# MadNLP/MadQP.jl

Measured on AMD Instinct MI355X. Metric: IPM iterations/sec (Mehrotra predictor-corrector, condensed KKT + Cholesky), dense QP fp64; value = steps / time of the timed iterations, initialize! excluded (value_reference_definition: iter / total_time), higher is better.
Workload: dtype f64

## Files before the change

__graft_entry__.py:

```python
import os
import subprocess
import sys

ROOT = os.path.dirname(os.path.abspath(__file__))
if ROOT not in sys.path:
    sys.path.insert(0, ROOT)


def build() -> None:
    subprocess.check_call(["make", "-C", os.path.join(ROOT, "madqp_jl_amd", "csrc"), "-j8"])
    subprocess.check_call(["make", "-C", os.path.join(ROOT, "tests", "csrc")])
    subprocess.check_call(["make", "-C", os.path.join(ROOT, "tests", "csrc_band")])
    subprocess.check_call(["make", "-C", os.path.join(ROOT, "tests", "csrc_solve")])
    import madqp_jl_amd as M

    lib = M.load_cdll()
    assert lib.madqp_version() == 100
    for name in M.EXPORTED_SYMBOLS:
        getattr(lib, name)


def smoke() -> None:
    import numpy as np

    import madqp_jl_amd as M
    from oracle import mpc
    from oracle import qp as Q

    be = M.HipBackend(0)
    qp = Q.synthetic_qp(20250614, 300, 120)
    dq = M.DeviceQP.from_numpy(be.device, qp.H, qp.q, qp.A, qp.lvar, qp.uvar, qp.lcon, qp.ucon, qp.x0)
    s = M.MPCSolver(dq, be, regularization=M.FixedRegularization(1e-8, -1e-8))
    r = s.solve()
    ref = mpc.solve(qp, kkt_system="condensed", regularization=mpc.FixedRegularization(1e-8, -1e-8))
    assert r["status"] == ref["status"] == M.SOLVE_SUCCEEDED, (r["status"], ref["status"])
    assert r["iter"] == ref["iter"], (r["iter"], ref["iter"])
    assert abs(r["objective"] - ref["objective"]) <= 1e-9 * max(1.0, abs(ref["objective"]))
    assert np.max(np.abs(r["solution"] - ref["solution"])) <= 1e-7
    for a, b in zip(r["trace"], ref["trace"]):
        tol = 1e-9 if min(a["mu"], b["mu"]) >= 1e-4 else 1e-6
        for k in ("alpha_p", "alpha_d", "inf_pr", "inf_du"):
            assert abs(a[k] - b[k]) <= tol * max(1.0, abs(b[k])), (a["k"], k, a[k], b[k])
    print(f"smoke ok: {r['iter']} iterations, objective {r['objective']:.12e}, "
          f"fp64 MFMA probe {be.probe_mfma_f64(100000):.1f} TFLOP/s")
    s.kkt.close()
    be.close()


if __name__ == "__main__":
    build()
    if len(sys.argv) > 1 and sys.argv[1] == "smoke":
        smoke()
```

madqp_jl_amd/csrc/chol.hip:

```cpp
#include <algorithm>
#include <cstdlib>

#include <vector>

#include "common.h"
#include "band_plan.inc"
#include "mid_plan.inc"
#include "solve_plan.inc"

typedef double double2_t __attribute__((ext_vector_type(2)));

namespace {
constexpr int NB = 128;
constexpr int NBO = 1024;
static_assert(SOLVE_NB == NB, "solve_plan.inc plans in this file's blocks");
constexpr int64_t SOLVE_MANY_MIN_DEFAULT = 32;
#ifndef P2_LDS_LD
#define P2_LDS_LD (NB + 1)
#endif
constexpr int LDS_LD = P2_LDS_LD;
constexpr int64_t WBLK = 2 * NB * NB;

typedef double double4_t __attribute__((ext_vector_type(4)));
#include "gemm_core.inc"
// ... 823 lines not shown
        }
}
template <int J>
__device__ __forceinline__ void ps16_step(double4_t (&z)[8], const double (&aw)[4], const double (&al)[7][4]) {
    double4_t t = {0.0, 0.0, 0.0, 0.0};
#pragma unroll
    for (int s = 0; s < 4; ++s) t = __builtin_amdgcn_mfma_f64_16x16x4f64(aw[s], z[J][s], t, 0, 0, 0);
    z[J] = t;
#pragma unroll
    for (int d = 0; d < 7; ++d)
        if (J + 1 + d < 8) {
#pragma unroll
            for (int s = 0; s < 4; ++s)
                z[J + 1 + d] = __builtin_amdgcn_mfma_f64_16x16x4f64(al[d][s], t[s], z[J + 1 + d], 0, 0, 0);
        }
}
__device__ __forceinline__ void panel_sub16_body(double* __restrict__ C, int64_t ld, const double* __restrict__ Lkk,
                                                 int64_t ldl, const double* __restrict__ Wcm, int64_t rows, int64_t rows_read) {
    const int lane = threadIdx.x & 63, wave = __builtin_amdgcn_readfirstlane(threadIdx.x >> 6);
    const int lo = lane & 15, hi = lane >> 4;
    const int64_t i0 = (int64_t)blockIdx.x * 64 + wave * 16;
    if (i0 >= rows) return;
    const int64_t gi = i0 + lo;
    const int64_t gir = gi < rows_read ? gi : rows_read - 1;
    double* Cp = C + gir + (int64_t)hi * ld;
    const double* Lq = Lkk + lo + (int64_t)hi * ldl;
    const double* Wq = Wcm + lo + hi * NB;
    double aw[3][4], al[3][7][4];
    ps16_load<0>(Lq, ldl, Wq, aw[0], al[0]);
    ps16_load<1>(Lq, ldl, Wq, aw[1], al[1]);
    double4_t z[8];
#pragma unroll
    for (int J = 0; J < 8; ++J)
#pragma unroll
        for (int v = 0; v < 4; ++v) z[J][v] = -Cp[(int64_t)(16 * J + 4 * v) * ld];
    ps16_load<2>(Lq, ldl, Wq, aw[2], al[2]);
    ps16_step<0>(z, aw[0], al[0]);
    ps16_load<3>(Lq, ldl, Wq, aw[0], al[0]);
    ps16_step<1>(z, aw[1], al[1]);
    ps16_load<4>(Lq, ldl, Wq, aw[1], al[1]);
    ps16_step<2>(z, aw[2], al[2]);
    ps16_load<5>(Lq, ldl, Wq, aw[2], al[2]);
    ps16_step<3>(z, aw[0], al[0]);
    ps16_load<6>(Lq, ldl, Wq, aw[0], al[0]);
    ps16_step<4>(z, aw[1], al[1]);
    ps16_load<7>(Lq, ldl, Wq, aw[1], al[1]);
    ps16_step<5>(z, aw[2], al[2]);
    ps16_step<6>(z, aw[0], al[0]);
    ps16_step<7>(z, aw[1], al[1]);
    if (gi < rows) {
        double* Co = C + gi + (int64_t)hi * ld;
#pragma unroll
        for (int J = 0; J < 8; ++J)
#pragma unroll
            for (int v = 0; v < 4; ++v) Co[(int64_t)(16 * J + 4 * v) * ld] = z[J][v];
    }
}

__global__ __launch_bounds__(256) void panel_sub16_kernel(double* __restrict__ C, int64_t ld, const double* __restrict__ Lkk,
                                                          int64_t ldl, const double* __restrict__ Wcm, int64_t rows,
                                                          int64_t rows_read, PanelBatch bt) {
    if (bt.list) {
        const int cnt = *bt.count;
        for (int pb = blockIdx.y; pb < cnt; pb += gridDim.y) {
            const int64_t b = bt.list[pb];
            panel_sub16_body(C + b * bt.sC, ld, Lkk + b * bt.sL, ldl, Wcm + b * bt.sW, rows, rows_read);
        }
        return;
    }
    if (gridDim.y > 1 || bt.skip) {
        const int64_t b = blockIdx.y;
        if (bt.skip && bt.skip[b] != 0) return;
        C += b * bt.sC;
        Lkk += b * bt.sL;
        Wcm += b * bt.sW;
    }
    panel_sub16_body(C, ld, Lkk, ldl, Wcm, rows, rows_read);
}

struct MidArgs {
    double* A;
    int64_t lda, n;
    int32_t nblk, k;
    const uint32_t* plan;
    double* winv;
    int32_t* info;
};
#ifdef MADQP_MID_STAMPS
__device__ unsigned long long madqp_mid_stamps[64][24];
#define MID_STAMP(slot)                                                                                              \
    do {                                                                                                             \
        if (threadIdx.x == 0 && blockIdx.x <= 2)                                                                     \
            madqp_mid_stamps[a.k & 63][8 * blockIdx.x + (slot)] = __builtin_amdgcn_s_memrealtime();                  \
    } while (0)
#else
#define MID_STAMP(slot)
#endif
constexpr int MID_THREADS = 512;

constexpr int XS_LD = 144;
static_assert(NB * XS_LD <= P2_S_DOUBLES + P2_WD_DOUBLES, "the operand image fits the diagonal kernel's LDS");
#ifdef MADQP_MID_STAMPS
#define DS_STAMP(slot)                                                                                   \
    do {                                                                                                 \
        if (threadIdx.x == 0) madqp_mid_stamps[kstep & 63][(slot)] = __builtin_amdgcn_s_memrealtime();   \
    } while (0)
#else
#define DS_STAMP(slot)
#endif
__device__ __forceinline__ void mid_diag_syrk(const double* __restrict__ Ckk, const double* __restrict__ R, int64_t lda, int nb,
                                              double* __restrict__ smem, int kstep) {
    const int tid = threadIdx.x, lane = tid & 63, wave = __builtin_amdgcn_readfirstlane(tid >> 6);
    const int lo = lane & 15, hi = lane >> 4;
    const int p = wave >> 1, first = (wave & 1) ? 5 : 0, cnt = (wave & 1) ? 4 : 5;
    int tI[5], tJ[5];
#pragma unroll
    for (int u = 0; u < 5; ++u) {
        int q = first + (u < cnt ? u : cnt - 1);
        tI[u] = (q <= p) ? p : 7 - p;
        tJ[u] = (q <= p) ? q : q - (p + 1);
    }
    double2_t rv[16];
#pragma unroll
    for (int q = 0; q < 16; ++q) {
        const int e = tid + MID_THREADS * q, c = e >> 6, i = 2 * (e & 63);
        rv[q] = *reinterpret_cast<const double2_t*>(R + i + (int64_t)c * lda);
    }
    double4_t acc[5];
#pragma unroll
    for (int u = 0; u < 5; ++u)
#pragma unroll
        for (int v = 0; v < 4; ++v) {
            int c = 16 * tJ[u] + hi + 4 * v;
            c = c < nb ? c : nb - 1;
            acc[u][v] = -Ckk[(16 * tI[u] + lo) + (int64_t)c * lda];
        }
#pragma unroll
    for (int q = 0; q < 16; ++q) {
        const int e = tid + MID_THREADS * q, c = e >> 6, i = 2 * (e & 63);
        *reinterpret_cast<double2_t*>(smem + c * XS_LD + i) = rv[q];
    }
    __syncthreads();
    DS_STAMP(4);
    const double* xa[5];
    const double* xb[5];
#pragma unroll
    for (int u = 0; u < 5; ++u) {
        xa[u] = smem + hi * XS_LD + 16 * tJ[u] + lo;
        xb[u] = smem + hi * XS_LD + 16 * tI[u] + lo;
    }
#pragma unroll 2
    for (int s4 = 0; s4 < 32; ++s4) {
#pragma unroll
        for (int u = 0; u < 5; ++u)
            acc[u] = __builtin_amdgcn_mfma_f64_16x16x4f64(xa[u][4 * s4 * XS_LD], xb[u][4 * s4 * XS_LD], acc[u], 0, 0, 0);
    }
    DS_STAMP(5);
    __syncthreads();
    DS_STAMP(6);
#pragma unroll
    for (int u = 0; u < 5; ++u) {
        if (u >= cnt) continue;
#pragma unroll
        for (int v = 0; v < 4; ++v) {
            const int r = 16 * tI[u] + lo, c = 16 * tJ[u] + hi + 4 * v;
            double x = -acc[u][v];
            if (r >= nb || c >= nb) x = (r == c) ? 1.0 : 0.0;
            smem[c * LDS_LD + r] = (r >= c) ? x : 0.0;
        }
    }
    __syncthreads();
}

__global__ __launch_bounds__(MID_THREADS) void chol_mid_step_kernel(MidArgs a) {
    __shared__ __attribute__((aligned(16))) double smem[P2_S_DOUBLES + P2_WD_DOUBLES];
    static_assert(P2_S_DOUBLES + P2_WD_DOUBLES >= 4 * TILE_DOUBLES, "the GEMM stages fit the diagonal kernel's LDS");
    const int tid = threadIdx.x, lane = tid & 63;
    const int wave = __builtin_amdgcn_readfirstlane(tid >> 6);
    const int k = a.k;
    MID_STAMP(0);
    if (blockIdx.x == 0) {
        const int64_t i0 = (int64_t)k * NB;
        const int nb = (int)((a.n - i0 < NB) ? (a.n - i0) : NB);
        double* Akk = a.A + i0 + i0 * a.lda;
        if (k > 0) mid_diag_syrk(Akk, a.A + i0 + (int64_t)(k - 1) * NB * a.lda, a.lda, nb, smem, k);
        MID_STAMP(1);
        MID_STAMP(2);
        double* Wcm = a.winv + (int64_t)k * WBLK;
        potf2_inv_body<MID_THREADS, 1>(Akk, a.lda, nb, Wcm, Wcm + NB * NB, a.info, (int32_t)i0, smem, smem + P2_S_DOUBLES,
                                       k > 0);
        MID_STAMP(3);
        return;
    }
    const uint32_t e = a.plan[(int)blockIdx.x - 1];
    const int bi = __builtin_amdgcn_readfirstlane((int)(e & 255u));
    const int bj = __builtin_amdgcn_readfirstlane((int)((e >> 8) & 255u));
    const int pan0 = __builtin_amdgcn_readfirstlane((int)((e >> 16) & 255u));
    const int kpan = __builtin_amdgcn_readfirstlane((int)(e >> 24));
    const int64_t i0 = (int64_t)bi * NB, j0 = (int64_t)bj * NB;
    if (wave >= 4) {
        const int nbar = kpan * (NB / BK) + 1;
        for (int b = 0; b < nbar; ++b) __builtin_amdgcn_s_barrier();
        return;
    }
    const int wi = wave & 1, wj = wave >> 1;
    const int lo = lane & 15, hi = lane >> 4;
    GemmArgs g{};
    g.X = a.A + (int64_t)pan0 * NB * a.lda;
    g.Y = g.X;
    g.ldx = g.ldy = a.lda;
    g.M = g.N = a.n;
    g.Mread = g.Nread = (int64_t)a.nblk * NB;
    g.K = kpan * NB;
    double4_t acc[4][4];
#pragma unroll
    for (int ti = 0; ti < 4; ++ti)
#pragma unroll
        for (int tj = 0; tj < 4; ++tj)
#pragma unroll
            for (int v = 0; v < 4; ++v) {
                int64_t gj = j0 + wj * 64 + tj * 16 + hi + 4 * v;
                gj = (gj < a.n) ? gj : a.n - 1;
                acc[ti][tj][v] = -a.A[i0 + wi * 64 + ti * 16 + lo + gj * a.lda];
            }
    mainloop_dma(g, i0, j0, smem, wi, wj, lane, wave, acc);
    MID_STAMP(1);
#pragma unroll
    for (int ti = 0; ti < 4; ++ti) {
        const int64_t gi = i0 + wi * 64 + ti * 16 + lo;
#pragma unroll
        for (int tj = 0; tj < 4; ++tj) {
#pragma unroll
            for (int v = 0; v < 4; ++v) {
                const int64_t gj = j0 + wj * 64 + tj * 16 + hi + 4 * v;
                if (gi < a.n && gj < a.n && gi >= gj) a.A[gi + gj * a.lda] = -acc[ti][tj][v];
            }
        }
    }
    MID_STAMP(7);
}

}

struct CholModes {
    bool sweep_upper;
    int32_t sweep_chunk;
    bool sweep_band;
    int64_t mid_max;
    int mid_cap;
    int64_t wt_min, wt_max;
    int64_t band_w;
};
static CholModes chol_modes_from_env() {
    auto num = [](const char* name, int64_t dflt) { return getenv(name) ? atoll(getenv(name)) : dflt; };
    auto on = [&](const char* name) { return num(name, 1) != 0; };
    CholModes m{};
    m.sweep_upper = on("MADQP_SWEEP_UPPER");
    m.sweep_chunk = (int32_t)std::max<int64_t>(1, num("MADQP_SWEEP_CHUNK", 64));
    m.sweep_band = on("MADQP_SWEEP_BAND");
    m.mid_max = num("MADQP_CHOL_MID_MAX", 13312);
    m.mid_cap = (int)num("MADQP_CHOL_MID_CAP", 0);
    m.wt_min = num("MADQP_CHOL_WMIN", 6);
    m.wt_max = num("MADQP_CHOL_WMAX", 20);
    m.band_w = std::max<int64_t>(0, num("MADQP_CHOL_BAND_W", 0));
    return m;
}
static const CholModes& chol_modes() {
    static const CholModes m = chol_modes_from_env();
    return m;
}

static hipError_t band_clear(madqp_chol* s) {
    const hipError_t e = s->mem.free_one(&s->band.d_jobs);
    s->band = madqp_chol_band{};
    s->band.extent = s->n - 1;
    return e;
}
static int32_t adopt_matrix(madqp_chol* s, double* A, int64_t lda) {
    ARG_TRY(s->ctx, A && lda >= (s->band.packed ? std::max<int64_t>(s->band.extent, 1) : s->n));
    s->A = A;
    s->lda = lda;
    s->upper_ok = false;
    return MADQP_OK;
}
static void forget_factor(madqp_chol* s) {
    s->A = nullptr;
    s->upper_ok = false;
}

extern "C" int32_t madqp_chol_create(madqp_ctx* ctx, int64_t n, madqp_chol** out) {
    ARG_TRY(ctx, ctx && out && n >= 0);
    *out = nullptr;
    madqp_chol* s = new (std::nothrow) madqp_chol();
    if (!s) return madqp_fail(ctx, MADQP_ERR_ALLOC, "host allocation failed");
    s->ctx = s->mem.ctx = ctx;
    s->n = s->npos = n;
    s->band.extent = n - 1;
    s->many_min = SOLVE_MANY_MIN_DEFAULT;
    const int64_t nblk = std::max<int64_t>(1, (n + NB - 1) / NB);
    const CholModes md = chol_modes_from_env();
    s->sweep_chunk = md.sweep_chunk;
    s->sweep_band = md.sweep_band;
    std::vector<int32_t> jobs;
    if (nblk - 1 > s->sweep_chunk && nblk < (1 << 20)) {
        s->sweep_maxc = (int32_t)band_sweep_jobs(nblk, -1, s->sweep_chunk, jobs);
        s->sweep_njobs = (int32_t)jobs.size();
    }
    s->tmp_len = nblk * NB + 2 * nblk * (int64_t)s->sweep_maxc * NB;
    s->utmp_len = nblk * NB + s->tmp_len;
    const bool with_x = nblk > 1 && nblk <= 160;
    const char* who = "madqp_chol_create";
    auto hip_ok = [&](hipError_t e) {
        return e == hipSuccess ? MADQP_OK : madqp_fail(ctx, MADQP_ERR_ALLOC, "madqp_chol_create(%lld): %s", (long long)n, hipGetErrorString(e));
    };
    int32_t r = s->mem.alloc(&s->winv, nblk * WBLK, who);
    if (!r) r = hip_ok(hipMemset(s->winv, 0, nblk * WBLK * sizeof(double)));
    double* scratch = nullptr;
    if (!r) r = s->mem.alloc(&scratch, with_x ? s->utmp_len : s->tmp_len, who);
    s->sweep_x = with_x ? scratch : nullptr;
    s->sweep_y = with_x && scratch ? scratch + nblk * NB : scratch;
    if (!r && !jobs.empty()) {
        r = s->mem.alloc(&s->d_jobs, (int64_t)jobs.size(), who);
        if (!r) r = hip_ok(hipMemcpy(s->d_jobs, jobs.data(), jobs.size() * sizeof(int32_t), hipMemcpyHostToDevice));
    }
    if (!r) r = s->mem.alloc(&s->d_info, 8, who);
    if (r) {
        madqp_chol_destroy(s);
        return r;
    }
    *out = s;
    return MADQP_OK;
}

static int64_t handle_plan(const madqp_chol* s, int64_t bw, std::vector<CholOp>& ops) {
    return chol_plan(s->n, bw < 0 ? s->n - 1 : bw, s->npos, s->ctx->gemm_slots, ops, chol_modes().wt_min, chol_modes().wt_max, chol_modes().band_w);
}

extern "C" int32_t madqp_chol_set_signature(madqp_chol* s, int64_t npos) {
    if (!s) return MADQP_ERR_ARG;
    ARG_TRY(s->ctx, npos >= 0 && npos <= s->n && (npos % NB == 0 || npos == s->n));
    ARG_TRY(s->ctx, s->band.bw < 0 || npos == s->n);
    s->npos = npos;
    s->plan.clear();
    return MADQP_OK;
}

extern "C" int32_t madqp_chol_destroy(madqp_chol* s) {
    if (!s) return MADQP_OK;
    (void)hipStreamSynchronize(s->ctx->stream);
    delete s;
    return MADQP_OK;
}

extern "C" int32_t madqp_chol_set_bandwidth(madqp_chol* s, int64_t bw) {
    if (!s) return MADQP_ERR_ARG;
    madqp_ctx* ctx = s->ctx;
    ARG_TRY(ctx, bw == -1 || (bw >= 0 && bw < s->n && s->npos == s->n));
    forget_factor(s);
    if (s->band.d_jobs) HIP_TRY(ctx, hipStreamSynchronize(ctx->stream));
    HIP_TRY(ctx, band_clear(s));
    s->plan.clear();
    if (bw < 0) return MADQP_OK;
    madqp_chol_band b;
    b.bw = bw;
    b.extent = handle_plan(s, bw, s->plan);
    if (s->sweep_band) {
        b.sweep_kb = band_sweep_blocks(bw);
        if (s->d_jobs) {
            std::vector<int32_t> jobs;
            band_sweep_jobs((s->n + NB - 1) / NB, b.sweep_kb, s->sweep_chunk, jobs);
            const size_t before = s->mem.owned.size();
            int32_t r = s->mem.alloc(&b.d_jobs, (int64_t)jobs.size(), "madqp_chol_set_bandwidth");
            const hipError_t e = r ? hipSuccess : hipMemcpy(b.d_jobs, jobs.data(), jobs.size() * sizeof(int32_t), hipMemcpyHostToDevice);
            if (e != hipSuccess) r = madqp_fail(ctx, MADQP_ERR_ALLOC, "madqp_chol_set_bandwidth: %s", hipGetErrorString(e));
            if (r) {
                s->mem.release(before);
                s->plan.clear();
                return r;
            }
            b.njobs = (int32_t)jobs.size();
        }
    }
    s->band = b;
    return MADQP_OK;
}

extern "C" int32_t madqp_chol_sweep_info(madqp_chol* s, int64_t* out_host) {
    if (!s || !out_host) return MADQP_ERR_ARG;
    const bool band = s->band.sweep_kb >= 0;
    const int64_t nblk = std::max<int64_t>(1, (s->n + NB - 1) / NB);
    out_host[0] = band ? s->band.sweep_kb : -1;
    out_host[1] = !s->d_jobs ? nblk : band ? s->band.njobs : s->sweep_njobs;
    out_host[2] = s->sweep_chunk;
    return MADQP_OK;
}

extern "C" int32_t madqp_chol_band_extent(madqp_chol* s, int64_t* extent_host) {
    if (!s) return MADQP_ERR_ARG;
    ARG_TRY(s->ctx, extent_host != nullptr);
    *extent_host = s->band.extent;
    return MADQP_OK;
}

static int64_t packed_ld_pad() {
    const char* e = getenv("MADQP_BAND_LD_PAD");
    return e ? std::max<int64_t>(0, atoll(e)) / 2 * 2 : BAND_PACKED_PAD;
}
extern "C" int32_t madqp_chol_packed_layout(madqp_chol* s, int64_t ld_in, int64_t* out_host) {
    if (!s) return MADQP_ERR_ARG;
    ARG_TRY(s->ctx, out_host != nullptr && s->band.bw >= 0);
    if (!band_packed_layout(s->n, s->band.extent, ld_in, out_host, packed_ld_pad()))
        return madqp_fail(s->ctx, MADQP_ERR_ARG, "madqp_chol_packed_layout: ld = %lld is below the extent %lld", (long long)ld_in,
                          (long long)s->band.extent);
    return MADQP_OK;
}
extern "C" int32_t madqp_chol_set_packed(madqp_chol* s, int32_t on) {
    if (!s) return MADQP_ERR_ARG;
    ARG_TRY(s->ctx, !on || (s->band.bw >= 0 && s->band.sweep_kb >= 0 && s->npos == s->n));
    if (s->band.packed != (on != 0)) forget_factor(s);
    s->band.packed = on != 0;
    return MADQP_OK;
}

static_assert(BAND_NB == NB && BAND_NBO == NBO, "chol_plan.inc plans in this file's blocks");

struct CholTarget {
    madqp_ctx* ctx;
    double* A;
    int64_t lda, n;
    double* winv;
    int32_t* info;
    bool batched = false;
    int64_t B = 1, sA = 0, sW = 0;
    const int32_t* skip = nullptr;
    const int32_t* list = nullptr;
    const int32_t* count = nullptr;
    bool packed = false;
    int64_t npad() const { return (n + NB - 1) / NB * NB; }
    bool padded() const { return packed || lda >= npad(); }
};
static int32_t target_gemm(const CholTarget& t, const GemmArgs& g, int cls, int64_t sY, int64_t sCin) {
    if (!t.batched) return madqp_gemm_tn(t.ctx, g, cls);
    const GemmBatch bt{t.B, t.sA, sY, t.sA, sCin, 0, t.skip, t.list, t.count};
    return madqp_gemm_tn(t.ctx, g, cls, nullptr, 0, &bt);
}

static int32_t panel_update(const CholTarget& t, const CholOp& o) {
    GemmArgs g{};
    g.X = t.A + o.row0 + o.k0 * t.lda;
    g.ldx = t.lda;
    g.Y = g.X;
    g.ldy = t.lda;
    g.C = t.A + o.row0 + o.row0 * t.lda;
    g.ldc = t.lda;
    g.Cin = g.C;
    g.ldcin = t.lda;
    g.alpha = (double)o.sign;
    g.beta = 1.0;
    g.M = o.rows;
    g.N = o.width;
    g.K = o.kend - o.k0;
    if (t.padded()) {
        g.Mread = (o.rows + NB - 1) / NB * NB;
        g.Nread = std::min<int64_t>(t.npad() - o.row0, (o.width + NB - 1) / NB * NB);
    }
    g.diag_off = 0;
    g.lower_only = 1;
    return target_gemm(t, g, MADQP_PROF_POTRF_GEMM, t.sA, t.sA);
}

static int32_t sweep_images(madqp_chol* s, double* A, int64_t lda, int64_t j0, int64_t w) {
    if (w <= 0) return MADQP_OK;
    madqp_ctx* ctx = s->ctx;
    ProfScope ps(ctx, MADQP_PROF_POTRF_DIAG);
    hipLaunchKernelGGL(sweep_image_kernel, dim3((unsigned)((w + NB - 1) / NB)), dim3(256), 0, ctx->stream, A, lda, s->n, j0, s->winv);
    LAUNCH_CHECK(ctx);
    return MADQP_OK;
}

static const auto sweep_fwd_kernel = trsv_fwd_sweep_kernel<false>;

int32_t madqp_chol_panel_solve(madqp_ctx* ctx, double* X, int64_t ldx, int64_t rows, int64_t rows_read, const double* L,
                               int64_t ldl, const double* Wcm, int64_t w, const CholTarget* batch) {
    if (rows <= 0) return MADQP_OK;
    ARG_TRY(ctx, w == NB);
    ARG_TRY(ctx, rows_read >= rows && (!batch || (batch->B >= 1 && batch->B <= 65535)));
    ProfScope ps(ctx, MADQP_PROF_POTRF_TRSM);
    const PanelBatch bt = batch ? PanelBatch{batch->sA, batch->sA, batch->sW, batch->skip, batch->list, batch->count}
                                : PanelBatch{0, 0, 0, nullptr};
    hipLaunchKernelGGL(panel_sub16_kernel, dim3((unsigned)((rows + 63) / 64), (unsigned)(batch ? batch->B : 1)), dim3(256), 0,
                       ctx->stream, X, ldx, L, ldl, Wcm, rows, rows_read, bt);
    LAUNCH_CHECK(ctx);
    return MADQP_OK;
}

static int32_t factor_block(const CholTarget& t, const CholOp& o) {
    madqp_ctx* ctx = t.ctx;
    const int64_t jb = o.row0, w = o.width, rows = o.rows;
    double* Ajj = t.A + jb + jb * t.lda;
    double* Wcm = t.winv + (jb / NB) * WBLK;
    {
        ProfScope ps(ctx, MADQP_PROF_POTRF_DIAG);
        const Potf2Batch bt = t.batched ? Potf2Batch{t.sA, t.sW, 1, t.skip, t.list, t.count} : Potf2Batch{0, 0, 0, nullptr};
        const auto diag_kernel = t.batched ? potf2_inv_kernel<0> : potf2_inv_kernel<1>;
        hipLaunchKernelGGL(diag_kernel, dim3((unsigned)t.B), dim3(P2_KTHREADS), 0, ctx->stream, Ajj, t.lda, (int)w, Wcm,
                           Wcm + NB * NB, t.info, (int32_t)jb, bt);
        LAUNCH_CHECK(ctx);
    }
    return madqp_chol_panel_solve(ctx, Ajj + w, t.lda, rows, t.padded() ? (rows + NB - 1) / NB * NB : rows, Ajj, t.lda, Wcm, w,
                                  t.batched ? &t : nullptr);
}

static int32_t run_ops(const CholTarget& t, const std::vector<CholOp>& ops) {
    for (const CholOp& o : ops) {
        const int32_t r = o.kind == CHOL_UPDATE ? panel_update(t, o) : factor_block(t, o);
        if (r) return r;
    }
    return MADQP_OK;
}
static CholTarget chol_target(madqp_chol* s, double* A, int64_t lda) {
    CholTarget t{s->ctx, A, lda, s->n, s->winv, s->d_info};
    t.packed = s->band.packed;
    return t;
}

static bool mid_plan_build(madqp_chol* s, int nblk, int cap) {
    MidPlan& mp = s->mid;
    if (mp.state) return mp.state > 0;
    mp.state = -1;
    if (nblk > 255 || cap < 1) return false;
    std::vector<std::vector<MidVisit>> steps;
    std::vector<int32_t> units;
    bool ok = false;
    for (int rounds = 1; rounds <= 64 && !ok; ++rounds) ok = mid_plan_steps(nblk, rounds * cap, steps, units, cap);
    if (!ok) return false;
    std::vector<uint32_t> w;
    std::vector<int32_t> count((size_t)nblk), first((size_t)nblk);
    for (int k = 0; k < nblk; ++k) {
        first[k] = (int32_t)w.size();
        mid_plan_units(nblk, k, steps[k], w);
        count[k] = (int32_t)w.size() - first[k];
        if (count[k] != units[k]) return false;
    }
    if (w.empty()) w.push_back(0);
    const size_t before = s->mem.owned.size();
    uint32_t* d_units = nullptr;
    if (s->mem.alloc(&d_units, (int64_t)w.size(), "madqp_chol_factor: mid-size plan") ||
        hipMemcpy(d_units, w.data(), w.size() * sizeof(uint32_t), hipMemcpyHostToDevice) != hipSuccess) {
        (void)hipGetLastError();
        s->mem.release(before);
        return false;
    }
    mp.count.swap(count);
    mp.first.swap(first);
    mp.d_units = d_units;
    mp.state = 1;
    return true;
}

static int32_t factor_mid(madqp_chol* s, double* A, int64_t lda) {
    madqp_ctx* ctx = s->ctx;
    const int64_t n = s->n;
    const int64_t npad_m = (n + NB - 1) / NB * NB;
    const int32_t nblk = (int32_t)(npad_m / NB);
    ProfScope ps_all(ctx, MADQP_PROF_POTRF_GEMM);
    ProfMute mute(ctx);
    for (int32_t k = 0; k < nblk; ++k) {
        hipLaunchKernelGGL(chol_mid_step_kernel, dim3((unsigned)(1 + s->mid.count[k])), dim3(MID_THREADS), 0, ctx->stream,
                           MidArgs{A, lda, n, nblk, k, s->mid.d_units + s->mid.first[k], s->winv, s->d_info});
        LAUNCH_CHECK(ctx);
        const int64_t jb = (int64_t)k * NB;
        const int32_t r = madqp_chol_panel_solve(ctx, A + (jb + NB) + jb * lda, lda, n - jb - NB, npad_m - jb - NB,
                                                 A + jb + jb * lda, lda, s->winv + (int64_t)k * WBLK, NB);
        if (r) return r;
    }
    const int32_t ri = sweep_images(s, A, lda, 0, n);
    if (ri) return ri;
    if (chol_modes().sweep_upper && s->sweep_x) {
        if (!s->upper) {
            const size_t before = s->mem.owned.size();
            if (s->mem.alloc(&s->upper, npad_m * npad_m, "madqp_chol_factor: U = L'")) {
                s->mem.release(before);
                return MADQP_OK;
            }
            s->upper_ld = npad_m;
        }
        hipLaunchKernelGGL(lower_to_upper_kernel, dim3(2 * nblk, 2 * nblk), dim3(256), 0, ctx->stream, A, lda, n, s->upper,
                           s->upper_ld);
        LAUNCH_CHECK(ctx);
        s->upper_ok = true;
    }
    return MADQP_OK;
}

static int32_t chol_factor_enqueue(madqp_chol* s, double* A, int64_t lda) {
    madqp_ctx* ctx = s->ctx;
    const int64_t n = s->n;
    HIP_TRY(ctx, hipMemsetAsync(s->d_info, 0, sizeof(int32_t), ctx->stream));
    const CholModes& md = chol_modes();
    if (s->band.bw < 0 && n <= md.mid_max && n > NB && s->npos == n && lda >= (n + NB - 1) / NB * NB && lda % 2 == 0 && (((uintptr_t)A) & 15) == 0 &&
        mid_plan_build(s, (int)((n + NB - 1) / NB), md.mid_cap > 0 ? md.mid_cap : ctx->gemm_slots / 2 - 1))
        return factor_mid(s, A, lda);
    if (s->plan.empty()) handle_plan(s, s->band.bw, s->plan);
    const int32_t r = run_ops(chol_target(s, A, lda), s->plan);
    if (r) return r;
    return sweep_images(s, A, lda, 0, n);
}

extern "C" int32_t madqp_chol_factor(madqp_chol* s, double* A, int64_t lda, int32_t* info_host) {
    if (!s) return MADQP_ERR_ARG;
    madqp_ctx* ctx = s->ctx;
    ARG_TRY(ctx, info_host != nullptr);
    int32_t r = adopt_matrix(s, A, lda);
    if (r) return r;
    *info_host = 0;
    if (s->n == 0) return MADQP_OK;
    if ((r = chol_factor_enqueue(s, A, lda))) return r;
    int32_t info = 0;
    HIP_TRY(ctx, hipMemcpyAsync(&info, s->d_info, sizeof(int32_t), hipMemcpyDeviceToHost, ctx->stream));
    HIP_TRY(ctx, hipStreamSynchronize(ctx->stream));
    *info_host = info;
    return MADQP_OK;
}

namespace {
__global__ void info_to_slot_kernel(const int32_t* __restrict__ info, double* __restrict__ slot) {
    *slot = (double)*info;
}
}
int32_t madqp_chol_factor_q(madqp_chol* s, double* A, int64_t lda, double* d_slot) {
    if (!s) return MADQP_ERR_ARG;
    madqp_ctx* ctx = s->ctx;
    ARG_TRY(ctx, d_slot != nullptr);
    int32_t r = adopt_matrix(s, A, lda);
    if (r) return r;
    if (s->n == 0) {
        HIP_TRY(ctx, hipMemsetAsync(d_slot, 0, sizeof(double), ctx->stream));
        return MADQP_OK;
    }
    if ((r = chol_factor_enqueue(s, A, lda))) return r;
    hipLaunchKernelGGL(info_to_slot_kernel, dim3(1), dim3(1), 0, ctx->stream, s->d_info, d_slot);
    LAUNCH_CHECK(ctx);
    return MADQP_OK;
}

int32_t madqp_chol_factor_batched(madqp_ctx* ctx, double* A, int64_t lda, int64_t n, int64_t sA, double* winv,
                                  int64_t sW, int32_t* info, int64_t B, const int32_t* skip, int64_t slots,
                                  const int32_t* list, const int32_t* count) {
    ARG_TRY(ctx, A && winv && info && lda >= n && B >= 1 && (!list || (count && slots >= 1)));
    if (n == 0) return MADQP_OK;
    HIP_TRY(ctx, hipMemsetAsync(info, 0, (size_t)B * sizeof(int32_t), ctx->stream));
    const CholTarget t{ctx, A, lda, n, winv, info, true, list ? slots : B, sA, sW, list ? nullptr : skip, list, count};
    std::vector<CholOp> ops;
    chol_plan_range(n, 0, n, ops);
    return run_ops(t, ops);
}

namespace {
__global__ void info_store_kernel(const int32_t* __restrict__ info, double* __restrict__ hdr) {
    hdr[0] = (double)*info;
    hdr[1] = 0.0;
}
constexpr int64_t PACK_HDR = 2;

bool panel_ok(const madqp_chol* s, int64_t j0, int64_t w) {
    return s->A && j0 >= 0 && w > 0 && j0 % NB == 0 && j0 + w <= s->n && (w % NB == 0 || j0 + w == s->n);
}
}

extern "C" int32_t madqp_chol_factor_begin(madqp_chol* s, double* A, int64_t lda) {
    if (!s) return MADQP_ERR_ARG;
    madqp_ctx* ctx = s->ctx;
    ARG_TRY(ctx, s->npos == s->n);
    ARG_TRY(ctx, s->band.bw < 0);
    if (const int32_t r = adopt_matrix(s, A, lda)) return r;
    HIP_TRY(ctx, hipMemsetAsync(s->d_info, 0, sizeof(int32_t), ctx->stream));
    return MADQP_OK;
}

extern "C" int32_t madqp_chol_factor_panel(madqp_chol* s, int64_t j0, int64_t w) {
    if (!s) return MADQP_ERR_ARG;
    ARG_TRY(s->ctx, panel_ok(s, j0, w) && s->band.bw < 0);
    std::vector<CholOp> ops;
    chol_plan_range(s->n, j0, w, ops);
    const int32_t r = run_ops(chol_target(s, s->A, s->lda), ops);
    return r ? r : sweep_images(s, s->A, s->lda, j0, w);
// ... 304 lines not shown
```

madqp_jl_amd/csrc/chol_plan.inc:

```
#include <algorithm>
#include <cassert>
#include <cstdint>
#include <vector>

constexpr int64_t BAND_NB = 128;
constexpr int64_t BAND_NBO = 1024;

enum { CHOL_UPDATE = 0, CHOL_BLOCK = 1 };
struct CholOp {
    int32_t kind;
    int64_t row0, rows, k0, kend, width;
    int32_t sign = -1;
};

static int64_t band_up(int64_t v) { return (v + BAND_NB - 1) / BAND_NB * BAND_NB; }
static int64_t band_down(int64_t v) { return v < 0 ? 0 : v / BAND_NB * BAND_NB; }

static int64_t plan_outer_width(int64_t rows, bool has_update, int64_t slots, int64_t wt_min, int64_t wt_max) {
    const int64_t mt = (rows + BAND_NB - 1) / BAND_NB;
    if (!has_update || mt <= 6) return BAND_NBO;
    int64_t best = BAND_NBO / BAND_NB;
    double best_eff = -1.0;
    for (int64_t wt = wt_min; wt <= wt_max && wt <= mt; ++wt) {
        const int64_t tiles = mt * wt - wt * (wt - 1) / 2;
        const int64_t rounds = (tiles + slots - 1) / slots;
        const double eff = (double)tiles / (double)(rounds * slots);
        if (eff > best_eff + 1e-9 || (eff > best_eff - 0.01 && wt > best && eff > 0.97)) {
            best_eff = std::max(eff, best_eff);
            best = wt;
        }
    }
    return best * BAND_NB;
}

static int64_t band_outer_width(int64_t rows, int64_t bw, bool has_update, int64_t slots, int64_t wt_min, int64_t wt_max,
                                int64_t force_wt) {
    const int64_t mt = (rows + BAND_NB - 1) / BAND_NB, mb = bw / BAND_NB + 1;
    if (mb >= mt) return plan_outer_width(rows, has_update, slots, wt_min, wt_max);
    if (force_wt > 0) return force_wt * BAND_NB;
    return std::max(wt_min, std::min(mb, wt_max)) * BAND_NB;
}

static void band_plan_block(int64_t n, int64_t bw, int64_t jb, int64_t w, std::vector<CholOp>& ops) {
    ops.push_back({CHOL_BLOCK, jb, std::min(band_up(bw), n - jb - w), 0, 0, w});
}
static void band_plan_update(int64_t n, int64_t bw, int64_t lo, int64_t hi, int64_t row0, int64_t width, int32_t sign,
                             std::vector<CholOp>& ops) {
    const int64_t k0 = std::max(lo, band_down(row0 - bw));
    if (k0 >= hi) return;
    ops.push_back({CHOL_UPDATE, row0, std::min(band_up(width + bw), n - row0), k0, hi, width, sign});
}
static void band_plan_range(int64_t n, int64_t bw, int64_t j0, int64_t w, std::vector<CholOp>& ops) {
    if (w <= BAND_NB) return band_plan_block(n, bw, j0, w, ops);
    const int64_t h = ((w + BAND_NB - 1) / BAND_NB + 1) / 2 * BAND_NB;
    band_plan_range(n, bw, j0, h, ops);
    band_plan_update(n, bw, j0, j0 + h, j0 + h, w - h, -1, ops);
    band_plan_range(n, bw, j0 + h, w - h, ops);
}

static void chol_plan_range(int64_t n, int64_t j0, int64_t w, std::vector<CholOp>& ops) {
    ops.clear();
    band_plan_range(n, n - 1, j0, w, ops);
}

static int64_t chol_plan(int64_t n, int64_t bw, int64_t npos, int64_t slots, std::vector<CholOp>& ops, int64_t wt_min = 6,
                         int64_t wt_max = 20, int64_t force_wt = 0) {
    assert(npos == n || bw == n - 1);
    ops.clear();
    int64_t W = 0;
    for (int64_t J0 = 0; J0 < n; J0 += W) {
        W = std::min<int64_t>(band_outer_width(n - J0, bw, J0 > 0, slots, wt_min, wt_max, force_wt), n - J0);
        if (J0 < npos && J0 + W > npos) W = npos - J0;
        if (J0 < npos) {
            band_plan_update(n, bw, 0, J0, J0, W, -1, ops);
        } else {
            band_plan_update(n, bw, 0, npos, J0, W, +1, ops);
            band_plan_update(n, bw, npos, J0, J0, W, -1, ops);
        }
        band_plan_range(n, bw, J0, W, ops);
    }
    int64_t extent = 0;
    for (const CholOp& o : ops)
        extent = std::max(extent, o.kind == CHOL_UPDATE ? o.row0 + o.rows - 1 - o.k0 : o.width + o.rows - 1);
    return extent;
}
```

madqp_jl_amd/csrc/common.h:

```cpp
#pragma once
#include <hip/hip_runtime.h>

#include <cstdarg>
#include <cstdint>
#include <cstdio>
#include <cstring>
#include <vector>

#include "../../include/madqp.h"

#define MADQP_RESULT_SLOTS 128
#define MADQP_FAULT_SLOT (MADQP_RESULT_SLOTS - 1)
#include "mpc_rules.inc"

struct ProfEvent {
    hipEvent_t a, b;
    int cls;
};

struct madqp_ctx {
    int device = 0;
    hipStream_t stream = nullptr;
    int64_t gemm_slots = 512;
    int64_t gemm_cap_slots = 0;
// ... 140 lines not shown
                       int prof_cls);
int32_t madqp_sparse_gram(madqp_ctx* ctx, int64_t n, const Csr& v, const Csr& vt, const double* w, const double* base,
                          int64_t ldbase, const double* dvec, const Csr& b, double* C, int64_t ldc);
int32_t madqp_sparse_gram_band(madqp_ctx* ctx, int64_t n, const Csr& v, const Csr& vt, const double* w, const double* dvec,
                               const Csr& b, double* C, int64_t ldc, int64_t bw, int64_t extent);

int32_t madqp_syrk_assemble_impl(madqp_ctx* ctx, int64_t n, int64_t kdim, const double* B, int64_t ldb, const double* w,
                                 const double* base, int64_t ldbase, const double* dvec, double* C, int64_t ldc);

struct DevOwner {
    madqp_ctx* ctx = nullptr;
    std::vector<void*> owned;
    DevOwner() = default;
    explicit DevOwner(madqp_ctx* c) : ctx(c) {}
    DevOwner(const DevOwner&) = delete;
    DevOwner& operator=(const DevOwner&) = delete;
    ~DevOwner() { release(); }
    template <class T>
    int32_t alloc(T** p, int64_t count, const char* who, bool zero = false) {
        *p = nullptr;
        const size_t bytes = (size_t)(count > 1 ? count : 1) * sizeof(T);
        hipError_t e = hipMalloc(p, bytes);
        if (e != hipSuccess) {
            *p = nullptr;
            (void)hipGetLastError();
            return madqp_fail(ctx, MADQP_ERR_ALLOC, "%s: hipMalloc(%zu): %s", who, bytes, hipGetErrorString(e));
        }
        owned.push_back(*p);
        if (zero && (e = hipMemsetAsync(*p, 0, bytes, ctx->stream)) != hipSuccess)
            return madqp_fail(ctx, MADQP_ERR_HIP, "%s: hipMemset: %s", who, hipGetErrorString(e));
        return MADQP_OK;
    }
    template <class T>
    int32_t grow(T** p, int64_t* have, int64_t want, const char* who) {
        if (*p && want <= *have) return MADQP_OK;
        if (*p) {
            (void)hipStreamSynchronize(ctx->stream);
            (void)free_one(p);
        }
        *have = 0;
        const int32_t r = alloc(p, want, who);
        if (!r) *have = want;
        return r;
    }
    void take(DevOwner& o) {
        owned.insert(owned.end(), o.owned.begin(), o.owned.end());
        o.owned.clear();
    }
    void release(size_t from = 0) {
        while (owned.size() > from) {
            (void)hipFree(owned.back());
            owned.pop_back();
        }
    }
    template <class T>
    hipError_t free_one(T** p) {
        for (size_t i = 0; i < owned.size(); ++i)
            if (owned[i] == *p) {
                owned.erase(owned.begin() + (std::ptrdiff_t)i);
                break;
            }
        const hipError_t e = *p ? hipFree(*p) : hipSuccess;
        *p = nullptr;
        return e;
    }
};

struct CholTarget;
int32_t madqp_chol_panel_solve(madqp_ctx* ctx, double* X, int64_t ldx, int64_t rows, int64_t rows_read, const double* L,
                               int64_t ldl, const double* Wcm, int64_t w, const CholTarget* batch = nullptr);
int32_t madqp_trsv_tile(madqp_ctx* ctx, int32_t trans, const double* L, int64_t ld, const double* winv, double* v,
                        int64_t w, double* tmp, int32_t* ctl);

struct madqp_chol_band {
    int64_t bw = -1;
    int64_t extent = 0;
    bool packed = false;
    int64_t sweep_kb = -1;
    int32_t* d_jobs = nullptr;
    int32_t njobs = 0;
};
struct MidPlan {
    int32_t state = 0;
    std::vector<int32_t> count, first;
    uint32_t* d_units = nullptr;
};

struct madqp_chol {
    madqp_ctx* ctx = nullptr;
    int64_t n = 0;
    DevOwner mem;
    double* winv = nullptr;
    double* sweep_x = nullptr;
    double* sweep_y = nullptr;
    int64_t tmp_len = 0, utmp_len = 0;
    int32_t* d_jobs = nullptr;
    int32_t sweep_chunk = 0, sweep_maxc = 0, sweep_njobs = 0;
    bool sweep_band = false;
    madqp_chol_band band;
    std::vector<struct CholOp> plan;
    int32_t* d_info = nullptr;
    double* A = nullptr;
    int64_t lda = 0;
    int64_t npos = 0;
    MidPlan mid;
    double* upper = nullptr;
    int64_t upper_ld = 0;
    bool upper_ok = false;
    double* many_ws = nullptr;
    int64_t many_ws_len = 0;
    int64_t many_min = 0;
};
```

madqp_jl_amd/csrc/mid_plan.inc:

```
#include <algorithm>
#include <cstdint>
#include <vector>

constexpr int MID_Q = 2;
struct MidVisit {
    int col, p0, q, units_before;
};
static bool mid_plan_steps(int nblk, int budget, std::vector<std::vector<MidVisit>>& steps, std::vector<int32_t>& units,
                           int round = 0) {
    if (round <= 0) round = budget;
    std::vector<int> upto(nblk, 0);
    steps.assign(nblk, {});
    units.assign(nblk, 0);
    struct Cand {
        int key, col, pend;
    };
    std::vector<Cand> cand;
    for (int k = 1; k < nblk; ++k) {
        cand.clear();
        for (int j = k; j < nblk; ++j) {
            const int pend = k - upto[j];
            if (pend <= 0) continue;
            const int key = (j <= k + 1) ? -100000 + j : (j - k) - (pend + MID_Q - 1) / MID_Q;
            cand.push_back({key, j, pend});
        }
        std::sort(cand.begin(), cand.end(), [](const Cand& x, const Cand& y) { return x.key != y.key ? x.key < y.key : x.col < y.col; });
        int all = 0;
        for (const Cand& c : cand) all += nblk - c.col - (c.col == k ? 1 : 0);
        const bool eager = all <= round;
        int u = 0;
        for (const Cand& c : cand) {
            const int h = nblk - c.col - (c.col == k ? 1 : 0);
            const bool forced = c.key <= 0;
            const int q = (c.col <= k + 1) ? c.pend : std::min(MID_Q, c.pend);
            if (!forced && !eager && (q < MID_Q || u + h > budget)) continue;
            if (q > MID_Q) return false;
            if (h > 0) steps[k].push_back({c.col, upto[c.col], q, u});
            u += h;
            upto[c.col] += q;
        }
        if (u > budget || upto[k] != k) return false;
        units[k] = u;
    }
    return true;
}

static void mid_plan_units(int nblk, int k, const std::vector<MidVisit>& visits, std::vector<uint32_t>& out) {
    std::vector<char> done(visits.size(), 0);
    for (size_t a = 0; a < visits.size(); ++a) {
        if (done[a]) continue;
        std::vector<int> cols;
        for (size_t b = a; b < visits.size(); ++b)
            if (!done[b] && visits[b].p0 == visits[a].p0 && visits[b].q == visits[a].q) {
                done[b] = 1;
                cols.push_back(visits[b].col);
            }
        std::sort(cols.begin(), cols.end());
        for (int i = cols.front(); i < nblk; ++i)
            for (int j : cols)
                if (j <= i && !(i == k && j == k))
                    out.push_back((uint32_t)i | (uint32_t)j << 8 | (uint32_t)visits[a].p0 << 16 | (uint32_t)visits[a].q << 24);
    }
}
```

Before: 0.7539.

## Factor large-matrix panels with windowed fused mid-step kernels

Extends the fused per-block-column Cholesky step kernel from small matrices to windows of large matrices. The planner recursively splits each panel width into windows of a few block columns, runs a trailing update between them, and factors each window with the scheduled mid-step kernel plus panel solves instead of the generic block/update ops. The unit encoding widens to 12-bit row indices with an offset so windows deep in large matrices fit. This aims to cut launch count and idle time in the factorization, and adds planning complexity and new index-packing limits.

```diff
diff --git a/__graft_entry__.py b/__graft_entry__.py
--- a/__graft_entry__.py
+++ b/__graft_entry__.py
@@ -12,6 +12,7 @@
     subprocess.check_call(["make", "-C", os.path.join(ROOT, "tests", "csrc")])
     subprocess.check_call(["make", "-C", os.path.join(ROOT, "tests", "csrc_band")])
     subprocess.check_call(["make", "-C", os.path.join(ROOT, "tests", "csrc_solve")])
+    subprocess.check_call(["make", "-C", os.path.join(ROOT, "tests", "csrc_window")])
     import madqp_jl_amd as M
 
     lib = M.load_cdll()
diff --git a/madqp_jl_amd/csrc/chol.hip b/madqp_jl_amd/csrc/chol.hip
--- a/madqp_jl_amd/csrc/chol.hip
+++ b/madqp_jl_amd/csrc/chol.hip
@@ -929,6 +929,7 @@
     double* A;
     int64_t lda, n;
     int32_t nblk, k;
+    int32_t o;
     const uint32_t* plan;
     double* winv;
     int32_t* info;
@@ -1030,20 +1031,20 @@
         const int64_t i0 = (int64_t)k * NB;
         const int nb = (int)((a.n - i0 < NB) ? (a.n - i0) : NB);
         double* Akk = a.A + i0 + i0 * a.lda;
-        if (k > 0) mid_diag_syrk(Akk, a.A + i0 + (int64_t)(k - 1) * NB * a.lda, a.lda, nb, smem, k);
+        if (k > a.o) mid_diag_syrk(Akk, a.A + i0 + (int64_t)(k - 1) * NB * a.lda, a.lda, nb, smem, k);
         MID_STAMP(1);
         MID_STAMP(2);
         double* Wcm = a.winv + (int64_t)k * WBLK;
         potf2_inv_body<MID_THREADS, 1>(Akk, a.lda, nb, Wcm, Wcm + NB * NB, a.info, (int32_t)i0, smem, smem + P2_S_DOUBLES,
-                                       k > 0);
+                                       k > a.o);
         MID_STAMP(3);
         return;
     }
-    const uint32_t e = a.plan[(int)blockIdx.x - 1];
-    const int bi = __builtin_amdgcn_readfirstlane((int)(e & 255u));
-    const int bj = __builtin_amdgcn_readfirstlane((int)((e >> 8) & 255u));
-    const int pan0 = __builtin_amdgcn_readfirstlane((int)((e >> 16) & 255u));
-    const int kpan = __builtin_amdgcn_readfirstlane((int)(e >> 24));
+    const MidUnit un = mid_unit_unpack(a.plan[(int)blockIdx.x - 1]);
+    const int bi = __builtin_amdgcn_readfirstlane(a.o + un.row);
+    const int bj = __builtin_amdgcn_readfirstlane(a.o + un.col);
+    const int pan0 = __builtin_amdgcn_readfirstlane(a.o + un.p0);
+    const int kpan = __builtin_amdgcn_readfirstlane(un.q);
     const int64_t i0 = (int64_t)bi * NB, j0 = (int64_t)bj * NB;
     if (wave >= 4) {
         const int nbar = kpan * (NB / BK) + 1;
@@ -1097,6 +1098,8 @@
     int mid_cap;
     int64_t wt_min, wt_max;
     int64_t band_w;
+    bool window;
+    int64_t window_wt;
 };
 static CholModes chol_modes_from_env() {
     auto num = [](const char* name, int64_t dflt) { return getenv(name) ? atoll(getenv(name)) : dflt; };
@@ -1110,6 +1113,8 @@
     m.wt_min = num("MADQP_CHOL_WMIN", 6);
     m.wt_max = num("MADQP_CHOL_WMAX", 20);
     m.band_w = std::max<int64_t>(0, num("MADQP_CHOL_BAND_W", 0));
+    m.window = on("MADQP_CHOL_WINDOW");
+    m.window_wt = std::max<int64_t>(0, num("MADQP_CHOL_WINDOW_WT", 8));
     return m;
 }
 static const CholModes& chol_modes() {
@@ -1179,8 +1184,10 @@
     return MADQP_OK;
 }
 
-static int64_t handle_plan(const madqp_chol* s, int64_t bw, std::vector<CholOp>& ops) {
-    return chol_plan(s->n, bw < 0 ? s->n - 1 : bw, s->npos, s->ctx->gemm_slots, ops, chol_modes().wt_min, chol_modes().wt_max, chol_modes().band_w);
+static int64_t handle_plan(const madqp_chol* s, int64_t bw, std::vector<CholOp>& ops, bool windows = false) {
+    const CholModes& md = chol_modes();
+    return chol_plan(s->n, bw < 0 ? s->n - 1 : bw, s->npos, s->ctx->gemm_slots, ops, md.wt_min, md.wt_max, md.band_w,
+                     !windows ? 0 : md.window_wt > 0 ? md.window_wt : -1);
 }
 
 extern "C" int32_t madqp_chol_set_signature(madqp_chol* s, int64_t npos) {
@@ -1189,6 +1196,7 @@
     ARG_TRY(s->ctx, s->band.bw < 0 || npos == s->n);
     s->npos = npos;
     s->plan.clear();
+    s->plan_windows = false;
     return MADQP_OK;
 }
 
@@ -1207,6 +1215,7 @@
     if (s->band.d_jobs) HIP_TRY(ctx, hipStreamSynchronize(ctx->stream));
     HIP_TRY(ctx, band_clear(s));
     s->plan.clear();
+    s->plan_windows = false;
     if (bw < 0) return MADQP_OK;
     madqp_chol_band b;
     b.bw = bw;
@@ -1283,6 +1292,7 @@
     const int32_t* list = nullptr;
     const int32_t* count = nullptr;
     bool packed = false;
+    const MidPlan* win = nullptr;
     int64_t npad() const { return (n + NB - 1) / NB * NB; }
     bool padded() const { return packed || lda >= npad(); }
 };
@@ -1358,9 +1368,37 @@
                                   t.batched ? &t : nullptr);
 }
 
+static int32_t window_steps(madqp_ctx* ctx, double* A, int64_t lda, int64_t n, int64_t j0, int64_t w, const MidPlan& mp, size_t index,
+                            double* winv, int32_t* info) {
+    const int64_t npad = (n + NB - 1) / NB * NB;
+    const int32_t nblk = (int32_t)(npad / NB), o = (int32_t)(j0 / NB), wt = (int32_t)((w + NB - 1) / NB);
+    ARG_TRY(ctx, mp.state > 0 && index + 1 < mp.win_first.size() && mp.win_first[index + 1] - mp.win_first[index] == wt);
+    for (int32_t k = 0; k < wt; ++k) {
+        const int32_t st = mp.win_first[index] + k;
+        {
+            ProfScope ps(ctx, MADQP_PROF_POTRF_GEMM);
+            hipLaunchKernelGGL(chol_mid_step_kernel, dim3((unsigned)(1 + mp.count[st])), dim3(MID_THREADS), 0, ctx->stream,
+                               MidArgs{A, lda, n, nblk, o + k, o, mp.d_units + mp.first[st], winv, info});
+            LAUNCH_CHECK(ctx);
+        }
+        const int64_t jb = (int64_t)(o + k) * NB;
+        const int32_t r = madqp_chol_panel_solve(ctx, A + (jb + NB) + jb * lda, lda, n - jb - NB, npad - jb - NB, A + jb + jb * lda, lda,
+                                                 winv + (int64_t)(o + k) * WBLK, NB);
+        if (r) return r;
+    }
+    return MADQP_OK;
+}
+
 static int32_t run_ops(const CholTarget& t, const std::vector<CholOp>& ops) {
+    size_t windows = 0;
     for (const CholOp& o : ops) {
-        const int32_t r = o.kind == CHOL_UPDATE ? panel_update(t, o) : factor_block(t, o);
+        int32_t r;
+        if (o.kind == CHOL_WINDOW) {
+            ARG_TRY(t.ctx, t.win && !t.batched && !t.packed);
+            r = window_steps(t.ctx, t.A, t.lda, t.n, o.row0, o.width, *t.win, windows++, t.winv, t.info);
+        } else {
+            r = o.kind == CHOL_UPDATE ? panel_update(t, o) : factor_block(t, o);
+        }
         if (r) return r;
     }
     return MADQP_OK;
@@ -1368,31 +1406,39 @@
 static CholTarget chol_target(madqp_chol* s, double* A, int64_t lda) {
     CholTarget t{s->ctx, A, lda, s->n, s->winv, s->d_info};
     t.packed = s->band.packed;
+    t.win = &s->win;
     return t;
 }
 
-static bool mid_plan_build(madqp_chol* s, int nblk, int cap) {
-    MidPlan& mp = s->mid;
+struct WindowShape {
+    int R, wt;
+};
+static bool step_plan_build(madqp_chol* s, MidPlan& mp, const std::vector<WindowShape>& shapes, int cap) {
     if (mp.state) return mp.state > 0;
     mp.state = -1;
-    if (nblk > 255 || cap < 1) return false;
+    if (cap < 1) return false;
     std::vector<std::vector<MidVisit>> steps;
     std::vector<int32_t> units;
-    bool ok = false;
-    for (int rounds = 1; rounds <= 64 && !ok; ++rounds) ok = mid_plan_steps(nblk, rounds * cap, steps, units, cap);
-    if (!ok) return false;
     std::vector<uint32_t> w;
-    std::vector<int32_t> count((size_t)nblk), first((size_t)nblk);
-    for (int k = 0; k < nblk; ++k) {
-        first[k] = (int32_t)w.size();
-        mid_plan_units(nblk, k, steps[k], w);
-        count[k] = (int32_t)w.size() - first[k];
-        if (count[k] != units[k]) return false;
-    }
+    std::vector<int32_t> count, first, win_first;
+    for (const WindowShape& sh : shapes) {
+        if (sh.wt > (1 << MID_COL_BITS) - 1 || sh.R > (1 << MID_ROW_BITS) - 1) return false;
+        bool ok = false;
+        for (int rounds = 1; rounds <= 64 && !ok; ++rounds) ok = mid_window_steps(sh.R, sh.wt, rounds * cap, steps, units, cap);
+        if (!ok) return false;
+        win_first.push_back((int32_t)count.size());
+        for (int k = 0; k < sh.wt; ++k) {
+            first.push_back((int32_t)w.size());
+            mid_window_units(sh.R, k, steps[k], w);
+            count.push_back((int32_t)w.size() - first.back());
+            if (count.back() != units[k]) return false;
+        }
+    }
+    win_first.push_back((int32_t)count.size());
     if (w.empty()) w.push_back(0);
     const size_t before = s->mem.owned.size();
     uint32_t* d_units = nullptr;
-    if (s->mem.alloc(&d_units, (int64_t)w.size(), "madqp_chol_factor: mid-size plan") ||
+    if (s->mem.alloc(&d_units, (int64_t)w.size(), "madqp_chol_factor: step plan") ||
         hipMemcpy(d_units, w.data(), w.size() * sizeof(uint32_t), hipMemcpyHostToDevice) != hipSuccess) {
         (void)hipGetLastError();
         s->mem.release(before);
@@ -1400,6 +1446,7 @@
     }
     mp.count.swap(count);
     mp.first.swap(first);
+    mp.win_first.swap(win_first);
     mp.d_units = d_units;
     mp.state = 1;
     return true;
@@ -1412,15 +1459,8 @@
     const int32_t nblk = (int32_t)(npad_m / NB);
     ProfScope ps_all(ctx, MADQP_PROF_POTRF_GEMM);
     ProfMute mute(ctx);
-    for (int32_t k = 0; k < nblk; ++k) {
-        hipLaunchKernelGGL(chol_mid_step_kernel, dim3((unsigned)(1 + s->mid.count[k])), dim3(MID_THREADS), 0, ctx->stream,
-                           MidArgs{A, lda, n, nblk, k, s->mid.d_units + s->mid.first[k], s->winv, s->d_info});
-        LAUNCH_CHECK(ctx);
-        const int64_t jb = (int64_t)k * NB;
-        const int32_t r = madqp_chol_panel_solve(ctx, A + (jb + NB) + jb * lda, lda, n - jb - NB, npad_m - jb - NB,
-                                                 A + jb + jb * lda, lda, s->winv + (int64_t)k * WBLK, NB);
-        if (r) return r;
-    }
+    const int32_t rw = window_steps(ctx, A, lda, n, 0, n, s->mid, 0, s->winv, s->d_info);
+    if (rw) return rw;
     const int32_t ri = sweep_images(s, A, lda, 0, n);
     if (ri) return ri;
     if (chol_modes().sweep_upper && s->sweep_x) {
@@ -1445,10 +1485,25 @@
     const int64_t n = s->n;
     HIP_TRY(ctx, hipMemsetAsync(s->d_info, 0, sizeof(int32_t), ctx->stream));
     const CholModes& md = chol_modes();
-    if (s->band.bw < 0 && n <= md.mid_max && n > NB && s->npos == n && lda >= (n + NB - 1) / NB * NB && lda % 2 == 0 && (((uintptr_t)A) & 15) == 0 &&
-        mid_plan_build(s, (int)((n + NB - 1) / NB), md.mid_cap > 0 ? md.mid_cap : ctx->gemm_slots / 2 - 1))
+    const int nblk = (int)((n + NB - 1) / NB), cap = md.mid_cap > 0 ? md.mid_cap : (int)(ctx->gemm_slots / 2 - 1);
+    const bool eligible = s->band.bw < 0 && !s->band.packed && n > NB && s->npos == n && lda >= (int64_t)nblk * NB && lda % 2 == 0 && (((uintptr_t)A) & 15) == 0;
+    if (eligible && n <= md.mid_max &&
+        step_plan_build(s, s->mid, {{nblk, nblk}}, cap))
         return factor_mid(s, A, lda);
-    if (s->plan.empty()) handle_plan(s, s->band.bw, s->plan);
+    bool windows = md.window && eligible;
+    if (windows && !s->win.state) {
+        std::vector<CholOp> ops;
+        handle_plan(s, -1, ops, true);
+        std::vector<WindowShape> shapes;
+        for (const CholOp& o : ops)
+            if (o.kind == CHOL_WINDOW) shapes.push_back({nblk - (int)(o.row0 / NB), (int)((o.width + NB - 1) / NB)});
+        step_plan_build(s, s->win, shapes, cap);
+    }
+    windows = windows && s->win.state > 0;
+    if (s->plan.empty() || s->plan_windows != windows) {
+        handle_plan(s, s->band.bw, s->plan, windows);
+        s->plan_windows = windows;
+    }
     const int32_t r = run_ops(chol_target(s, A, lda), s->plan);
     if (r) return r;
     return sweep_images(s, A, lda, 0, n);
diff --git a/madqp_jl_amd/csrc/chol_plan.inc b/madqp_jl_amd/csrc/chol_plan.inc
--- a/madqp_jl_amd/csrc/chol_plan.inc
+++ b/madqp_jl_amd/csrc/chol_plan.inc
@@ -6,7 +6,7 @@
 constexpr int64_t BAND_NB = 128;
 constexpr int64_t BAND_NBO = 1024;
 
-enum { CHOL_UPDATE = 0, CHOL_BLOCK = 1 };
+enum { CHOL_UPDATE = 0, CHOL_BLOCK = 1, CHOL_WINDOW = 2 };
 struct CholOp {
     int32_t kind;
     int64_t row0, rows, k0, kend, width;
@@ -58,14 +58,26 @@
     band_plan_range(n, bw, j0 + h, w - h, ops);
 }
 
+static void chol_plan_windows(int64_t n, int64_t j0, int64_t w, int64_t window_wt, std::vector<CholOp>& ops) {
+    if (window_wt < 0 || w <= window_wt * BAND_NB) {
+        ops.push_back({CHOL_WINDOW, j0, n - j0, 0, 0, w});
+        return;
+    }
+    const int64_t h = ((w + BAND_NB - 1) / BAND_NB + 1) / 2 * BAND_NB;
+    chol_plan_windows(n, j0, h, window_wt, ops);
+    band_plan_update(n, n - 1, j0, j0 + h, j0 + h, w - h, -1, ops);
+    chol_plan_windows(n, j0 + h, w - h, window_wt, ops);
+}
+
 static void chol_plan_range(int64_t n, int64_t j0, int64_t w, std::vector<CholOp>& ops) {
     ops.clear();
     band_plan_range(n, n - 1, j0, w, ops);
 }
 
 static int64_t chol_plan(int64_t n, int64_t bw, int64_t npos, int64_t slots, std::vector<CholOp>& ops, int64_t wt_min = 6,
-                         int64_t wt_max = 20, int64_t force_wt = 0) {
+                         int64_t wt_max = 20, int64_t force_wt = 0, int64_t window_wt = 0) {
     assert(npos == n || bw == n - 1);
+    assert(window_wt == 0 || (npos == n && bw == n - 1));
     ops.clear();
     int64_t W = 0;
     for (int64_t J0 = 0; J0 < n; J0 += W) {
@@ -77,10 +89,13 @@
             band_plan_update(n, bw, 0, npos, J0, W, +1, ops);
             band_plan_update(n, bw, npos, J0, J0, W, -1, ops);
         }
-        band_plan_range(n, bw, J0, W, ops);
+        if (window_wt != 0)
+            chol_plan_windows(n, J0, W, window_wt, ops);
+        else
+            band_plan_range(n, bw, J0, W, ops);
     }
     int64_t extent = 0;
     for (const CholOp& o : ops)
-        extent = std::max(extent, o.kind == CHOL_UPDATE ? o.row0 + o.rows - 1 - o.k0 : o.width + o.rows - 1);
+        extent = std::max(extent, o.kind == CHOL_UPDATE ? o.row0 + o.rows - 1 - o.k0 : o.kind == CHOL_WINDOW ? o.rows - 1 : o.width + o.rows - 1);
     return extent;
 }
diff --git a/madqp_jl_amd/csrc/common.h b/madqp_jl_amd/csrc/common.h
--- a/madqp_jl_amd/csrc/common.h
+++ b/madqp_jl_amd/csrc/common.h
@@ -246,6 +246,7 @@
 };
 struct MidPlan {
     int32_t state = 0;
+    std::vector<int32_t> win_first;
     std::vector<int32_t> count, first;
     uint32_t* d_units = nullptr;
 };
@@ -263,6 +264,8 @@
     bool sweep_band = false;
     madqp_chol_band band;
     std::vector<struct CholOp> plan;
+    bool plan_windows = false;
+    MidPlan win;
     int32_t* d_info = nullptr;
     double* A = nullptr;
     int64_t lda = 0;
diff --git a/madqp_jl_amd/csrc/mid_plan.inc b/madqp_jl_amd/csrc/mid_plan.inc
--- a/madqp_jl_amd/csrc/mid_plan.inc
+++ b/madqp_jl_amd/csrc/mid_plan.inc
@@ -6,46 +6,63 @@
 struct MidVisit {
     int col, p0, q, units_before;
 };
-static bool mid_plan_steps(int nblk, int budget, std::vector<std::vector<MidVisit>>& steps, std::vector<int32_t>& units,
-                           int round = 0) {
+static bool mid_window_steps(int R, int wt, int budget, std::vector<std::vector<MidVisit>>& steps, std::vector<int32_t>& units,
+                             int round = 0) {
+    if (wt < 1 || R < wt) return false;
     if (round <= 0) round = budget;
-    std::vector<int> upto(nblk, 0);
-    steps.assign(nblk, {});
-    units.assign(nblk, 0);
+    std::vector<int> upto(wt, 0);
+    steps.assign(wt, {});
+    units.assign(wt, 0);
     struct Cand {
         int key, col, pend;
     };
     std::vector<Cand> cand;
-    for (int k = 1; k < nblk; ++k) {
+    for (int k = 1; k < wt; ++k) {
         cand.clear();
-        for (int j = k; j < nblk; ++j) {
+        for (int j = k; j < wt; ++j) {
             const int pend = k - upto[j];
             if (pend <= 0) continue;
             const int key = (j <= k + 1) ? -100000 + j : (j - k) - (pend + MID_Q - 1) / MID_Q;
             cand.push_back({key, j, pend});
         }
         std::sort(cand.begin(), cand.end(), [](const Cand& x, const Cand& y) { return x.key != y.key ? x.key < y.key : x.col < y.col; });
-        int all = 0;
-        for (const Cand& c : cand) all += nblk - c.col - (c.col == k ? 1 : 0);
+        int64_t all = 0;
+        for (const Cand& c : cand) all += R - c.col - (c.col == k ? 1 : 0);
         const bool eager = all <= round;
-        int u = 0;
+        int64_t u = 0;
         for (const Cand& c : cand) {
-            const int h = nblk - c.col - (c.col == k ? 1 : 0);
+            const int h = R - c.col - (c.col == k ? 1 : 0);
             const bool forced = c.key <= 0;
             const int q = (c.col <= k + 1) ? c.pend : std::min(MID_Q, c.pend);
             if (!forced && !eager && (q < MID_Q || u + h > budget)) continue;
             if (q > MID_Q) return false;
-            if (h > 0) steps[k].push_back({c.col, upto[c.col], q, u});
+            if (h > 0) steps[k].push_back({c.col, upto[c.col], q, (int)u});
             u += h;
             upto[c.col] += q;
         }
         if (u > budget || upto[k] != k) return false;
-        units[k] = u;
+        units[k] = (int32_t)u;
     }
     return true;
 }
+static bool mid_plan_steps(int nblk, int budget, std::vector<std::vector<MidVisit>>& steps, std::vector<int32_t>& units,
+                           int round = 0) {
+    return mid_window_steps(nblk, nblk, budget, steps, units, round);
+}
 
-static void mid_plan_units(int nblk, int k, const std::vector<MidVisit>& visits, std::vector<uint32_t>& out) {
+struct MidUnit {
+    int row, col, p0, q;
+};
+constexpr int MID_ROW_BITS = 12, MID_COL_BITS = 8;
+constexpr uint32_t mid_unit_pack(const MidUnit& u) {
+    return (uint32_t)u.row | (uint32_t)u.col << MID_ROW_BITS | (uint32_t)u.p0 << (MID_ROW_BITS + MID_COL_BITS) |
+           (uint32_t)u.q << (MID_ROW_BITS + 2 * MID_COL_BITS);
+}
+constexpr MidUnit mid_unit_unpack(uint32_t e) {
+    return {(int)(e & ((1u << MID_ROW_BITS) - 1)), (int)((e >> MID_ROW_BITS) & ((1u << MID_COL_BITS) - 1)),
+            (int)((e >> (MID_ROW_BITS + MID_COL_BITS)) & ((1u << MID_COL_BITS) - 1)), (int)(e >> (MID_ROW_BITS + 2 * MID_COL_BITS))};
+}
+static void mid_window_units(int R, int k, const std::vector<MidVisit>& visits, std::vector<uint32_t>& out) {
     std::vector<char> done(visits.size(), 0);
     for (size_t a = 0; a < visits.size(); ++a) {
         if (done[a]) continue;
@@ -56,9 +73,16 @@
                 cols.push_back(visits[b].col);
             }
         std::sort(cols.begin(), cols.end());
-        for (int i = cols.front(); i < nblk; ++i)
+        for (int i = cols.front(); i < R; ++i)
             for (int j : cols)
-                if (j <= i && !(i == k && j == k))
-                    out.push_back((uint32_t)i | (uint32_t)j << 8 | (uint32_t)visits[a].p0 << 16 | (uint32_t)visits[a].q << 24);
+                if (j <= i && !(i == k && j == k)) out.push_back(mid_unit_pack({i, j, visits[a].p0, visits[a].q}));
     }
 }
+static void mid_plan_units(int nblk, int k, const std::vector<MidVisit>& visits, std::vector<uint32_t>& out) {
+    std::vector<uint32_t> w;
+    mid_window_units(nblk, k, visits, w);
+    for (uint32_t e : w) {
+        const MidUnit u = mid_unit_unpack(e);
+        out.push_back((uint32_t)u.row | (uint32_t)u.col << 8 | (uint32_t)u.p0 << 16 | (uint32_t)u.q << 24);
+    }
+}
```

After: 0.7611 (median of 6 runs). About the same (+0.9%).
